# mandanasmi/lane-slam

Hardware: AMD Instinct MI355X
Metric: frames/sec (640x480) detect->descript->project->sanity->associate (higher is better)
Workload: dtype u8/f64 (FP4 e2m1 MFMA with exact f32 accumulation for association)

## Files before the change

### include/lanefront.h

```cpp
#ifndef LANEFRONT_H
#define LANEFRONT_H

#include <stddef.h>
#include <stdint.h>

#define LF_API __attribute__((visibility("default")))

#ifdef __cplusplus
extern "C" {
#endif

#define LF_ABI_VERSION 5

typedef enum lf_status {
    LF_OK = 0,
    LF_ERR_BAD_ARG = -1,
    LF_ERR_CAPACITY = -2,
    LF_ERR_HIP = -3,
    LF_ERR_NOT_INITIALISED = -4,
    LF_ERR_UNSUPPORTED = -5,
    LF_ERR_DECODE = -6
} lf_status;

#define LF_WHITE 0
// ... 399 lines not shown
LF_API int lf_jpeg_decode_batch_gpu_async(lf_handle* h, const uint8_t* const* jpeg, const size_t* jpeg_size, int n_frames,
                                   int rows, int cols, uint8_t* frames_device, int n_threads);
LF_API int lf_jpeg_status(lf_handle* h, int* frame_status, int n_frames, int* n_failed);
LF_API int lf_jpeg_decode_for_detect_async(lf_handle* h, const uint8_t* const* jpeg, const size_t* jpeg_size, int n_frames, int n_threads);
LF_API int lf_jpeg_info(const uint8_t* jpeg, size_t jpeg_size, int* rows, int* cols, int* components, int* hmax, int* vmax);
LF_API int lf_frames_buffer(lf_handle* h, uint8_t** device_ptr, size_t* bytes);

#define LF_MSG_DETECTOR 0
#define LF_MSG_GROUND 1
#define LF_MSG_FILTERED 2
LF_API int lf_serialize_segments(lf_handle* h, const lf_segments* segs, int segs_on_device, int n_frames, int stage,
                          uint8_t* out, size_t out_capacity, int out_on_device, int64_t* frame_byte_offset);
LF_API int lf_deserialize_segments(lf_handle* h, const uint8_t* bodies, int bodies_on_device, const int64_t* frame_byte_offset,
                            int n_frames, lf_segments* out, int out_on_device, int* n_segments);

LF_API int lf_draw_lines(lf_handle* h, int n_frames, const lf_segments* seg, int seg_on_device, uint8_t* out_bgr, int out_on_device);
LF_API int lf_draw_lines_image(lf_handle* h, const uint8_t* bgr, int n_frames, int rows, int cols, const lf_segments* seg, int seg_on_device,
                               uint8_t* out_bgr, int images_on_device);

#define LF_JPEG_ENCODE_STAGES 8
LF_API size_t lf_jpeg_encode_bound(int rows, int cols);
LF_API int lf_jpeg_encode_batch(lf_handle* h, const uint8_t* bgr, int bgr_on_device, int n_frames, int rows, int cols, int quality, uint8_t* out,
                                size_t out_stride, uint32_t* out_size, int out_on_device);
LF_API int lf_jpeg_encode_timing(lf_handle* h, double* ms_per_stage, int n);
LF_API const char* lf_jpeg_encode_stage_name(int stage);

#define LF_RECTIFY_STAGES 1
LF_API int lf_set_camera(lf_handle* h, const double* K, const double* D, const double* R, const double* P, int cam_w, int cam_h);
LF_API int lf_set_rectified_input(lf_handle* h, int flag);
LF_API int lf_get_rectified_input(lf_handle* h, int* flag);
LF_API int lf_rectify_map(lf_handle* h, float* mapx, float* mapy);
LF_API int lf_rectify_batch(lf_handle* h, const uint8_t* src, int src_on_device, int n_frames, int rows, int cols, int channels, uint8_t* dst,
                            int dst_on_device);
LF_API int lf_rectify_timing(lf_handle* h, double* ms_per_stage, int n);
LF_API const char* lf_rectify_stage_name(int stage);

typedef enum lf_buffer_id {
    LF_BUF_BGR = 0,
    LF_BUF_MASKS = 1,
    LF_BUF_EDGES = 2,
    LF_BUF_LSD_ANGLE = 3,
    LF_BUF_LSD_MODGRAD = 4,
    LF_BUF_LSD_ORDER = 5,
    LF_BUF_LSD_NORDER = 6,
    LF_BUF_LBD_DX = 7,
    LF_BUF_LBD_DY = 8,
    LF_BUF_LSD_COUNTS = 9,
    LF_BUF_LSD_SCRATCH = 10,
    LF_BUF_LSD_NLOW = 11
} lf_buffer_id;
LF_API int lf_debug_fetch(lf_handle* h, int buffer_id, void* dst, size_t bytes);
LF_API int lf_debug_detmath(lf_handle* h, int which, const double* a, const double* b_or_null, double* y, int n);
LF_API int lf_debug_probe(lf_handle* h, int width, int write, size_t bytes, int reps);
LF_API int lf_debug_lsd_binary(lf_handle* h, const uint8_t* img, int rows, int cols, float* lines4, int cap, int* n_out);
LF_API int lf_debug_std_sort(lf_handle* h, const int32_t* keys, int n, int32_t* order);
LF_API int lf_lsd_size(const lf_handle* h, int* rows, int* cols);
LF_API int lf_suggested_depth(const lf_handle* h);

LF_API int lf_lsd_list_capacity(const lf_handle* h, int* entries, int* grown);
LF_API int lf_lsd_scratch_stride(const lf_handle* h);

#define LF_N_STAGES 16
LF_API int lf_set_profiling(lf_handle* h, int enabled);
LF_API int lf_get_timing(lf_handle* h, double* ms_per_stage, int32_t* launches_per_stage, int n);
LF_API int lf_reset_timing(lf_handle* h);
LF_API const char* lf_stage_name(int stage);

#ifdef __cplusplus
}
#endif
#endif
```

### lane_slam_amd/_lib.py

```python
import ctypes
import os

from .config import LfConfig

_HERE = os.path.dirname(os.path.abspath(__file__))
SO_PATH = os.environ.get("LANEFRONT_LIBRARY") or os.path.join(_HERE, "liblanefront.so")

LF_N_STAGES = 16
LF_MAP_N_STAGES = 4
LF_MSG_DETECTOR, LF_MSG_GROUND, LF_MSG_FILTERED = 0, 1, 2
(LF_BUF_BGR, LF_BUF_MASKS, LF_BUF_EDGES, LF_BUF_LSD_ANGLE, LF_BUF_LSD_MODGRAD, LF_BUF_LSD_ORDER,
 LF_BUF_LSD_NORDER, LF_BUF_LBD_DX, LF_BUF_LBD_DY, LF_BUF_LSD_COUNTS, LF_BUF_LSD_SCRATCH, LF_BUF_LSD_NLOW) = range(12)

EXPORTS = (
    "lf_abi_version", "lf_create", "lf_destroy", "lf_last_error", "lf_synchronize", "lf_get_stream",
    "lf_set_image", "lf_detect_lines", "lf_process_batch", "lf_process_batch_async", "lf_wait", "lf_associate", "lf_associate_float", "lf_kmeans",
    "lf_jpeg_decode_batch", "lf_jpeg_info", "lf_frames_buffer", "lf_serialize_segments", "lf_deserialize_segments",
    "lf_debug_fetch", "lf_debug_detmath", "lf_debug_probe", "lf_debug_lsd_binary", "lf_lsd_size", "lf_set_profiling", "lf_get_timing", "lf_reset_timing", "lf_stage_name",
    "lf_map_create", "lf_map_destroy", "lf_map_last_error", "lf_map_get_stream", "lf_map_synchronize", "lf_map_seed", "lf_map_size",
    "lf_map_associate", "lf_map_pack_block", "lf_map_update", "lf_map_step", "lf_map_step_host", "lf_map_fetch",
    "lf_map_set_profiling", "lf_map_get_timing", "lf_map_stage_name",
    "lf_descriptor_default_params", "lf_set_descriptor_params", "lf_get_descriptor_params",
    "lf_edlines_default_params", "lf_keylines_batch", "lf_describe_keylines", "lf_keylines_debug_fetch", "lf_set_image_edlines", "lf_knn_match", "lf_radius_match", "lf_jpeg_decode_batch_gpu", "lf_jpeg_decode_batch_gpu_async", "lf_jpeg_status", "lf_jpeg_decode_for_detect_async",
    "lf_set_tie_rule", "lf_map_set_tie_rule", "lf_debug_std_sort", "lf_suggested_depth", "lf_lsd_list_capacity", "lf_lsd_scratch_stride", "lf_set_detector", "lf_detector_failures", "lf_keylines_batch_async", "lf_keylines_frame_status", "lf_lsd_keylines_batch", "lf_select_queries",
    "lf_lsd_default_options", "lf_lsd_keylines_batch_ex", "lf_keylines_batch_masked",
    "lf_matcher_add", "lf_matcher_clear", "lf_matcher_size", "lf_matcher_match", "lf_matcher_knn_match", "lf_matcher_radius_match",
    "lf_lane_filter_default_config", "lf_lane_filter_create", "lf_lane_filter_destroy", "lf_lane_filter_last_error", "lf_lane_filter_grid",
    "lf_lane_filter_set_tables", "lf_lane_filter_reset", "lf_lane_filter_step", "lf_lane_filter_get_poses", "lf_lane_filter_get_belief",
    "lf_lane_filter_synchronize", "lf_lane_filter_set_profiling", "lf_lane_filter_get_timing", "lf_lane_filter_stage_name",
    "lf_hough_default_params", "lf_set_hough_params", "lf_get_hough_params",
    "lf_dense_default_params", "lf_set_dense_params", "lf_get_dense_params",
    "lf_ai_transform_batch", "lf_set_ai_transform", "lf_get_ai_transform",
    "lf_draw_lines", "lf_draw_lines_image",
    "lf_jpeg_encode_bound", "lf_jpeg_encode_batch", "lf_jpeg_encode_timing", "lf_jpeg_encode_stage_name",
    "lf_set_camera", "lf_set_rectified_input", "lf_get_rectified_input", "lf_rectify_map", "lf_rectify_batch", "lf_rectify_timing",
    "lf_rectify_stage_name",
    "lf_map_default_view", "lf_map_bounds", "lf_map_render", "lf_map_render_counts", "lf_map_render_timing", "lf_map_render_stage_name",
    "lf_sizeof_camera_view", "lf_map_camera_view", "lf_map_render_camera", "lf_map_render_camera_timing",
    "lf_sizeof_align_config", "lf_sizeof_align_result", "lf_map_align_default_config", "lf_map_align", "lf_map_step_aligned",
    "lf_map_step_aligned_host", "lf_map_align_timing",
    "lf_sizeof_smooth_config", "lf_map_smooth_default_config", "lf_map_smooth", "lf_map_step_smoothed", "lf_map_step_smoothed_host",
    "lf_map_smooth_timing",
    "lf_sizeof_localize_config", "lf_sizeof_localize_result", "lf_map_localize_default_config", "lf_map_localize", "lf_map_localize_timing",
    "lf_sizeof_prune_config", "lf_sizeof_prune_result", "lf_map_prune_default_config", "lf_map_prune", "lf_map_prune_timing",
)
LF_ALIGN_OK, LF_ALIGN_FEW, LF_ALIGN_DEGENERATE, LF_ALIGN_REJECTED = 0, 1, 2, 3
ALIGN_STATUS = ("ok", "few", "degenerate", "rejected")
LF_MAP_RENDER_STAGES = 4
LF_JPEG_ENCODE_STAGES = 8
LF_RECTIFY_STAGES = 1
LF_LANE_FILTER_PREDICT, LF_LANE_FILTER_UPDATE = 1, 2
LF_LANE_FILTER_MAX_CELLS = 4096
LF_LANE_FILTER_N_STAGES = 2
LANE_FILTER_PARAMS = ("mean_d_0", "mean_phi_0", "sigma_d_0", "sigma_phi_0", "delta_d", "delta_phi", "d_max", "d_min", "phi_max",
                      "phi_min", "cov_v", "linewidth_white", "linewidth_yellow", "lanewidth", "min_max", "sigma_d_mask", "sigma_phi_mask")
DETECTORS = {"lsd": 0, "edlines": 1, "hough": 2, "dense": 3}
HOUGH_KEYS = ("hough_threshold", "hough_min_line_length", "hough_max_line_gap")
DENSE_KEYS = ("sobel_threshold",)
TIE_RULES = {"lowest": 0, "mihasher": 1}
LF_MAX_OCTAVES = 5


class LfSegments(ctypes.Structure):
    _fields_ = [
        ("capacity", ctypes.c_int32),
        ("frame_offset", ctypes.c_void_p),
        ("lines", ctypes.c_void_p), ("normals", ctypes.c_void_p), ("color", ctypes.c_void_p),
        ("pixels_normalized", ctypes.c_void_p), ("ground", ctypes.c_void_p), ("keep", ctypes.c_void_p),
        ("desc", ctypes.c_void_p), ("code", ctypes.c_void_p),
    ]

# ... 146 lines not shown
    lib.lf_process_batch_async.restype = ci
    lib.lf_wait.argtypes = [vp, ctypes.POINTER(ci)]
    lib.lf_wait.restype = ci
    lib.lf_associate.argtypes = [vp, vp, ci, vp, ci, vp, vp, ci]
    lib.lf_associate_float.argtypes = [vp, vp, ci, vp, ci, vp, vp, ci]
    lib.lf_kmeans.argtypes = [vp, vp, ci, ci, ci, vp, ci, ctypes.c_double, vp, vp, vp, vp]
    lib.lf_ai_transform_batch.argtypes = [vp, vp, ci, ci, ci, ci, vp]
    lib.lf_set_ai_transform.argtypes = [vp, vp, vp]
    lib.lf_get_ai_transform.argtypes = [vp, vp, vp]
    lib.lf_draw_lines.argtypes = [vp, ci, ctypes.POINTER(LfSegments), ci, vp, ci]
    lib.lf_draw_lines_image.argtypes = [vp, vp, ci, ci, ci, ctypes.POINTER(LfSegments), ci, vp, ci]
    lib.lf_jpeg_encode_bound.argtypes = [ci, ci]
    lib.lf_jpeg_encode_bound.restype = ctypes.c_size_t
    lib.lf_jpeg_encode_batch.argtypes = [vp, vp, ci, ci, ci, ci, ci, vp, ctypes.c_size_t, vp, ci]
    lib.lf_jpeg_encode_batch.restype = ci
    lib.lf_jpeg_encode_timing.argtypes = [vp, vp, ci]
    lib.lf_jpeg_encode_timing.restype = ci
    lib.lf_jpeg_encode_stage_name.argtypes = [ci]
    lib.lf_jpeg_encode_stage_name.restype = ctypes.c_char_p
    lib.lf_set_camera.argtypes = [vp, vp, vp, vp, vp, ci, ci]
    lib.lf_set_rectified_input.argtypes = [vp, ci]
    lib.lf_get_rectified_input.argtypes = [vp, ctypes.POINTER(ci)]
    lib.lf_rectify_map.argtypes = [vp, vp, vp]
    lib.lf_rectify_batch.argtypes = [vp, vp, ci, ci, ci, ci, ci, vp, ci]
    lib.lf_rectify_timing.argtypes = [vp, vp, ci]
    for f in ("lf_set_camera", "lf_set_rectified_input", "lf_get_rectified_input", "lf_rectify_map", "lf_rectify_batch", "lf_rectify_timing"):
        getattr(lib, f).restype = ci
    lib.lf_rectify_stage_name.argtypes = [ci]
    lib.lf_rectify_stage_name.restype = ctypes.c_char_p
    lib.lf_jpeg_decode_batch.argtypes = [vp, ctypes.POINTER(vp), ctypes.POINTER(ctypes.c_size_t), ci, ci, ci, vp, ci, ci,
                                         ctypes.POINTER(ci)]
    lib.lf_jpeg_decode_batch.restype = ci
    lib.lf_jpeg_decode_batch_gpu.argtypes = lib.lf_jpeg_decode_batch.argtypes
    lib.lf_jpeg_decode_batch_gpu.restype = ci
    lib.lf_jpeg_decode_batch_gpu_async.argtypes = [vp, ctypes.POINTER(vp), ctypes.POINTER(ctypes.c_size_t), ci, ci, ci, vp, ci]
    lib.lf_jpeg_decode_batch_gpu_async.restype = ci
    lib.lf_jpeg_status.argtypes = [vp, ctypes.POINTER(ci), ci, ctypes.POINTER(ci)]
    lib.lf_jpeg_decode_for_detect_async.argtypes = [vp, ctypes.POINTER(vp), ctypes.POINTER(ctypes.c_size_t), ci, ci]
    lib.lf_jpeg_decode_for_detect_async.restype = ci
    lib.lf_jpeg_status.restype = ci
    lib.lf_jpeg_info.argtypes = [vp, ctypes.c_size_t] + [ctypes.POINTER(ci)] * 5
    lib.lf_jpeg_info.restype = ci
    lib.lf_frames_buffer.argtypes = [vp, ctypes.POINTER(vp), ctypes.POINTER(ctypes.c_size_t)]
    lib.lf_frames_buffer.restype = ci
    lib.lf_serialize_segments.argtypes = [vp, ctypes.POINTER(LfSegments), ci, ci, ci, vp, ctypes.c_size_t, ci,
                                          ctypes.POINTER(ctypes.c_int64)]
    lib.lf_serialize_segments.restype = ci
    lib.lf_deserialize_segments.argtypes = [vp, vp, ci, ctypes.POINTER(ctypes.c_int64), ci, ctypes.POINTER(LfSegments), ci,
                                            ctypes.POINTER(ci)]
    lib.lf_deserialize_segments.restype = ci
    lib.lf_debug_fetch.argtypes = [vp, ci, vp, ctypes.c_size_t]
    lib.lf_debug_detmath.argtypes = [vp, ci, vp, vp, vp, ci]
    lib.lf_debug_detmath.restype = ci
    lib.lf_debug_probe.argtypes = [vp, ci, ci, ctypes.c_size_t, ci]
    lib.lf_debug_probe.restype = ci
    lib.lf_debug_lsd_binary.argtypes = [vp, vp, ci, ci, vp, ci, ctypes.POINTER(ci)]
    lib.lf_debug_lsd_binary.restype = ci
    lib.lf_lsd_size.argtypes = [vp, ctypes.POINTER(ci), ctypes.POINTER(ci)]
    lib.lf_set_profiling.argtypes = [vp, ci]
    lib.lf_get_timing.argtypes = [vp, vp, vp, ci]
    lib.lf_reset_timing.argtypes = [vp]
    lib.lf_stage_name.argtypes = [ci]
    lib.lf_stage_name.restype = ctypes.c_char_p
    i64p = ctypes.POINTER(ctypes.c_int64)
    lib.lf_map_create.argtypes = [ci, ctypes.POINTER(LfMapConfig), ctypes.POINTER(vp)]
    lib.lf_map_destroy.argtypes = [vp]
    lib.lf_map_destroy.restype = None
    lib.lf_map_last_error.argtypes = [vp]
    lib.lf_map_last_error.restype = ctypes.c_char_p
    lib.lf_map_get_stream.argtypes = [vp, ctypes.POINTER(vp)]
    lib.lf_map_synchronize.argtypes = [vp]
    lib.lf_map_seed.argtypes = [vp, vp, vp, vp, ci, ci]
    lib.lf_map_size.argtypes = [vp, ctypes.POINTER(ci), ctypes.POINTER(ci), i64p, i64p]
    lib.lf_map_associate.argtypes = [vp, vp, vp, vp, ci, vp, vp, ci]
    lib.lf_map_pack_block.argtypes = [vp, vp, ctypes.POINTER(LfSegments), ci, ci, vp, vp, vp, ci, vp, ci]
    lib.lf_map_update.argtypes = [vp, vp, ci, ci]
    lib.lf_map_step.argtypes = [vp, vp, ctypes.POINTER(LfSegments), ci, ci, vp, ci, vp, vp]
    lib.lf_map_step_host.argtypes = [vp, ctypes.POINTER(LfSegments), ci, ci, vp, ci, vp, vp]
    lib.lf_map_step_host.restype = ci
    lib.lf_map_fetch.argtypes = [vp, ci, ci, vp, vp, vp, vp, vp]
    lib.lf_map_set_profiling.argtypes = [vp, ci]
    lib.lf_map_set_profiling.restype = ci
    lib.lf_map_get_timing.argtypes = [vp, vp, vp, ci]
    lib.lf_map_get_timing.restype = ci
    lib.lf_map_stage_name.argtypes = [ci]
    lib.lf_map_stage_name.restype = ctypes.c_char_p
    lib.lf_map_default_view.argtypes = [ctypes.POINTER(LfMapView)]
    lib.lf_map_default_view.restype = None
    lib.lf_map_bounds.argtypes = [vp, ctypes.POINTER(LfMapView), vp, ctypes.POINTER(ci)]
    lib.lf_map_render.argtypes = [vp, ctypes.POINTER(LfMapView), vp, ci, vp, ci, ctypes.POINTER(ci), ctypes.POINTER(ci)]
    lib.lf_map_render_counts.argtypes = [vp, ctypes.POINTER(ci), ctypes.POINTER(ci)]
    lib.lf_map_render_timing.argtypes = [vp, vp, ci]
    for f in ("lf_map_bounds", "lf_map_render", "lf_map_render_counts", "lf_map_render_timing"):
        getattr(lib, f).restype = ci
    lib.lf_map_render_stage_name.argtypes = [ci]
    lib.lf_map_render_stage_name.restype = ctypes.c_char_p
    lib.lf_sizeof_camera_view.argtypes = []
    lib.lf_map_camera_view.argtypes = [vp, ci, ci, ci, ci, ci, ctypes.POINTER(LfCameraView)]
    lib.lf_map_render_camera.argtypes = [vp, ctypes.POINTER(LfCameraView), vp, ci, vp, vp, ci, vp]
    lib.lf_map_render_camera_timing.argtypes = [vp, vp, ci]
    for f in ("lf_sizeof_camera_view", "lf_map_camera_view", "lf_map_render_camera", "lf_map_render_camera_timing"):
        getattr(lib, f).restype = ci
    lib.lf_sizeof_align_config.argtypes = []
    lib.lf_sizeof_align_result.argtypes = []
    lib.lf_map_align_default_config.argtypes = [ctypes.POINTER(LfAlignConfig)]
    lib.lf_map_align_default_config.restype = None
# ... 137 lines not shown
```

### lane_slam_amd/csrc/k_canny.hip

```cpp
#include "common.h"

namespace lf {

#ifndef LF_CANNY_ROWS
#define LF_CANNY_ROWS 62
#endif
constexpr int CB_R = LF_CANNY_ROWS;
static_assert(CB_R + 2 <= 64, "the columns beside a strip are worked out with one lane per magnitude row");

typedef short cn_s2 __attribute__((ext_vector_type(2)));

struct CannyH {
    cn_s2 d_br, s_br;
    int d_g, s_g;
};
struct CannyG {
    cn_s2 dx_br, dy_br;
    int dx_g, dy_g;
    uint32_t m_br;
    int m_g;
};

__device__ __forceinline__ cn_s2 canny_a_plus_2b(cn_s2 a, cn_s2 b)
{
    cn_s2 d;
    const uint32_t two = 0x00020002u;
    asm("v_pk_mad_i16 %0, %1, %2, %3" : "=v"(d) : "v"(b), "v"(two), "v"(a));
    return d;
}

__device__ __forceinline__ CannyH canny_hterms(uint32_t aL, uint32_t aM, uint32_t aR)
{
    const cn_s2 l = __builtin_bit_cast(cn_s2, aL & 0x00ff00ffu), m = __builtin_bit_cast(cn_s2, aM & 0x00ff00ffu), r = __builtin_bit_cast(cn_s2, aR & 0x00ff00ffu);
    const int lg = (int)((aL >> 8) & 0xffu), mg = (int)((aM >> 8) & 0xffu), rg = (int)((aR >> 8) & 0xffu);
    CannyH h;
    h.d_br = r - l;
    h.s_br = canny_a_plus_2b(l, m) + r;
    h.d_g = rg - lg;
    h.s_g = lg + 2 * mg + rg;
    return h;
}

__device__ __forceinline__ int canny_mag_at(const uint32_t* __restrict__ img, int W, int Hc, int x, int y)
{
    if (x < 0 || x >= W || y < 0 || y >= Hc) return 0;
    const int xl = max(x - 1, 0), xr = min(x + 1, W - 1), yu = max(y - 1, 0), yd = min(y + 1, Hc - 1);
    const uint32_t a00 = img[(size_t)yu * W + xl], a01 = img[(size_t)yu * W + x], a02 = img[(size_t)yu * W + xr];
    const uint32_t a10 = img[(size_t)y * W + xl], a12 = img[(size_t)y * W + xr];
    const uint32_t a20 = img[(size_t)yd * W + xl], a21 = img[(size_t)yd * W + x], a22 = img[(size_t)yd * W + xr];
    int best = 0;
#pragma unroll
    for (int ch = 0; ch < 3; ++ch) {
        const int sh = 8 * ch;
        const int v00 = (a00 >> sh) & 255, v01 = (a01 >> sh) & 255, v02 = (a02 >> sh) & 255, v10 = (a10 >> sh) & 255, v12 = (a12 >> sh) & 255;
        const int v20 = (a20 >> sh) & 255, v21 = (a21 >> sh) & 255, v22 = (a22 >> sh) & 255;
        const int dx = (v02 - v00) + 2 * (v12 - v10) + (v22 - v20);
        const int dy = (v20 - v00) + 2 * (v21 - v01) + (v22 - v02);
        best = max(best, abs(dx) + abs(dy));
    }
    return best;
}

__device__ __forceinline__ int canny_from_left(int v, int edge) { return __builtin_amdgcn_update_dpp(edge, v, 0x138, 0xf, 0xf, false); }
__device__ __forceinline__ int canny_from_right(int v, int edge) { return __builtin_amdgcn_update_dpp(edge, v, 0x130, 0xf, 0xf, false); }

struct CannyBand {
    const uint32_t* img;
    __amdgpu_buffer_rsrc_t rsrc;
    __amdgpu_buffer_rsrc_t rs_weak, rs_strong;
    int W, Hc, Ww, low, high;
    int x0, y0, y_end;
    uint32_t xl, xm, xr;
    int lane;
    bool in_image;
    bool st_ok;
    uint32_t st_off;
    int* halo;
};

__device__ __forceinline__ void canny_fetch(const CannyBand& c, int prow, uint32_t (&px)[3])
{
    const int yy = min(max(prow, 0), c.Hc - 1);
    const int row = yy * c.W * 4;
    px[0] = __builtin_amdgcn_raw_buffer_load_b32(c.rsrc, (int)c.xl, row, 0);
    px[1] = __builtin_amdgcn_raw_buffer_load_b32(c.rsrc, (int)c.xm, row, 0);
    px[2] = __builtin_amdgcn_raw_buffer_load_b32(c.rsrc, (int)c.xr, row, 0);
}

__device__ __forceinline__ void canny_halo_chunk(const CannyBand& c, int t)
{
    const int side = c.lane >> 5, j = t - 4 + (c.lane & 31);
    if ((c.lane & 31) < 18 && j >= 0 && j < 64)
        c.halo[side * 64 + j] = canny_mag_at(c.img, c.W, c.Hc, side ? c.x0 + 64 : c.x0 - 1, c.y0 - 1 + j);
    __builtin_amdgcn_fence(__ATOMIC_RELEASE, "wavefront");
    __builtin_amdgcn_wave_barrier();
}

template <int A, int B, int C>
__device__ __forceinline__ void canny_step(const CannyBand& c, int t, uint32_t (&px)[3][3], CannyH (&H)[3], int (&M)[3], CannyG (&G)[3])
{
    const int p = c.y0 - 2 + t;
    if ((t & 15) == 0) canny_halo_chunk(c, t);
    H[C] = canny_hterms(px[C][0], px[C][1], px[C][2]);
    canny_fetch(c, p + 3, px[C]);
    if (t < 2) return;
    {
        const int y = p - 1;
        const cn_s2 zero = { 0, 0 };
        CannyG g;
        g.dx_br = canny_a_plus_2b(H[A].d_br, H[B].d_br) + H[C].d_br;
        g.dy_br = H[C].s_br - H[A].s_br;
        g.dx_g = H[A].d_g + 2 * H[B].d_g + H[C].d_g;
        g.dy_g = H[C].s_g - H[A].s_g;
        const cn_s2 m_br = __builtin_elementwise_max(g.dx_br, zero - g.dx_br) + __builtin_elementwise_max(g.dy_br, zero - g.dy_br);
        g.m_g = abs(g.dx_g) + abs(g.dy_g);
        g.m_br = __builtin_bit_cast(uint32_t, m_br);
        const int best = max(max((int)(g.m_br & 0xffffu), (int)(g.m_br >> 16)), g.m_g);
        M[C] = (c.in_image && y >= 0 && y < c.Hc) ? best : 0;
        G[C] = g;
    }
    const int yn = p - 2;
    if (yn < c.y0 || yn >= c.y_end) return;
    const int m = M[B];
    const unsigned long long over = __ballot(m > c.low);
    unsigned long long keep = 0ull, hi = 0ull;
    if (over != 0ull) {
        const int* hl = c.halo + (yn - c.y0 + 1);
        const int up = M[A], dn = M[C];
        const int mL = canny_from_left(m, hl[0]), mR = canny_from_right(m, hl[64]);
        const int upL = canny_from_left(up, hl[-1]), upR = canny_from_right(up, hl[63]);
        const int dnL = canny_from_left(dn, hl[1]), dnR = canny_from_right(dn, hl[65]);
        const CannyG g = G[B];
        const int m_b = (int)(g.m_br & 0xffffu), m_r = (int)(g.m_br >> 16);
        const bool take_g = g.m_g > m_b;
        const bool take_r = m_r > max(m_b, g.m_g);
        const int xs = take_r ? (int)g.dx_br.y : (take_g ? g.dx_g : (int)g.dx_br.x);
        const int ys = take_r ? (int)g.dy_br.y : (take_g ? g.dy_g : (int)g.dy_br.x);
        const int TG22 = (int)(0.4142135623730950488016887242097 * (1 << 15) + 0.5);
        const int ax = abs(xs), ay = abs(ys) << 15;
        int tg22x;
        asm("v_mul_u32_u24 %0, %1, %2" : "=v"(tg22x) : "v"(ax), "v"(TG22));
        const int tg67x = tg22x + (ax << 16);
        const bool neg = (xs ^ ys) < 0;
        const unsigned long long keep_h = __ballot(m > mL) & __ballot(m >= mR);
        const unsigned long long keep_v = __ballot(m > up) & __ballot(m >= dn);
        const unsigned long long keep_d = __ballot(m > (neg ? upR : upL)) & __ballot(m > (neg ? dnL : dnR));
        const unsigned long long is_h = __ballot(ay < tg22x), is_v = __ballot(ay > tg67x) & ~is_h;
        keep = over & ((is_h & keep_h) | (is_v & keep_v) | (~(is_h | is_v) & keep_d));
        hi = keep & __ballot(m > c.high);
    }
    if (c.st_ok) {
        const int o = (yn * c.Ww + (c.x0 >> 5)) * 4;
        const bool second = c.lane != 0;
        __builtin_amdgcn_raw_buffer_store_b32(second ? (uint32_t)(keep >> 32) : (uint32_t)keep, c.rs_weak, (int)c.st_off, o, 0);
        __builtin_amdgcn_raw_buffer_store_b32(second ? (uint32_t)(hi >> 32) : (uint32_t)hi, c.rs_strong, (int)c.st_off, o, 0);
    }
}

#ifndef LF_CANNY_WAVES
#define LF_CANNY_WAVES 7
#endif
__global__ __launch_bounds__(256) __attribute__((amdgpu_waves_per_eu(LF_CANNY_WAVES, LF_CANNY_WAVES))) void k_canny_nms(CannyParams p, int n_units, int n_strips, int n_bands,
                                                   const uint32_t* __restrict__ bgr, uint32_t* __restrict__ strong,
                                                   uint32_t* __restrict__ weak)
{
    __shared__ int halo[4][128];
    int b = (int)blockIdx.x;
    {
        const int per_frame = (n_strips * n_bands + 3) / 4;
        const int full = (n_units / (n_strips * n_bands)) / 8 * 8 * per_frame;
        if (b < full) {
            const int grp = b / (8 * per_frame), r = b - grp * 8 * per_frame;
            b = (grp * 8 + (r & 7)) * per_frame + (r >> 3);
        }
    }
    const int wave = __builtin_amdgcn_readfirstlane((int)(threadIdx.x >> 6));
    const int per_frame_u = n_strips * n_bands, wg_per_frame = (per_frame_u + 3) / 4;
    const int f = b / wg_per_frame, uf = (b - f * wg_per_frame) * 4 + wave;
    if (uf >= per_frame_u || f * per_frame_u >= n_units) return;
    const int u = uf;
    CannyBand c;
    c.lane = (int)(threadIdx.x & 63u);
    const int strip = u % n_strips, band = u / n_strips;
    c.W = p.W; c.Hc = p.Hc; c.Ww = p.Ww; c.low = p.low; c.high = p.high;
    c.img = bgr + (size_t)f * p.Hc * p.W;
    c.rsrc = __builtin_amdgcn_make_buffer_rsrc(const_cast<uint32_t*>(c.img), 0, p.Hc * p.W * 4, 0x00020000);
    c.rs_weak = __builtin_amdgcn_make_buffer_rsrc(weak + (size_t)f * p.Hc * p.Ww, 0, p.Hc * p.Ww * 4, 0x00020000);
    c.rs_strong = __builtin_amdgcn_make_buffer_rsrc(strong + (size_t)f * p.Hc * p.Ww, 0, p.Hc * p.Ww * 4, 0x00020000);
    c.x0 = strip * 64; c.y0 = band * CB_R; c.y_end = min(c.y0 + CB_R, p.Hc);
    const int x = c.x0 + c.lane;
    c.in_image = x < p.W;
    c.st_ok = c.lane < 2 && (c.x0 >> 5) + c.lane < p.Ww;
    c.st_off = 4u * (uint32_t)c.lane;
    const int xm = min(x, p.W - 1);
    c.xm = 4u * (uint32_t)xm; c.xl = 4u * (uint32_t)max(xm - 1, 0); c.xr = 4u * (uint32_t)min(xm + 1, p.W - 1);
    c.halo = halo[threadIdx.x >> 6];
    uint32_t px[3][3];
    CannyH H[3];
    int M[3] = { 0, 0, 0 };
    CannyG G[3];
    canny_fetch(c, c.y0 - 2, px[0]);
    canny_fetch(c, c.y0 - 1, px[1]);
    canny_fetch(c, c.y0, px[2]);
    const int steps = (c.y_end - c.y0) + 4;
    for (int t = 0; t < steps; t += 3) {
        canny_step<1, 2, 0>(c, t, px, H, M, G);
        canny_step<2, 0, 1>(c, t + 1, px, H, M, G);
        canny_step<0, 1, 2>(c, t + 2, px, H, M, G);
    }
}

void launch_canny(const CannyParams& p, const uint32_t* bgr, int n_frames, uint32_t* strong, uint32_t* weak,
                  hipStream_t s)
{
    const int n_strips = (p.W + 63) / 64, n_bands = (p.Hc + CB_R - 1) / CB_R;
    const int n_units = n_strips * n_bands * n_frames;
    const int wg_per_frame = (n_strips * n_bands + 3) / 4;
    hipLaunchKernelGGL(k_canny_nms, dim3(wg_per_frame * n_frames), dim3(256), 0, s, p, n_units, n_strips, n_bands, bgr, strong, weak);
}

__device__ __forceinline__ uint32_t fill_up(uint32_t w, uint32_t s) { return (((w + s) ^ w) & w) | s; }

__global__ __launch_bounds__(1024) void k_hysteresis(CannyParams p, uint32_t* __restrict__ strong,
                                                      const uint32_t* __restrict__ weak)
{
    extern __shared__ uint32_t lds[];
    const int nw = p.Hc * p.Ww;
    uint32_t* S = lds;
    uint32_t* Wk = lds + nw;
    const int f = blockIdx.x;
    uint32_t* gs = strong + (size_t)f * nw;
    const uint32_t* gw = weak + (size_t)f * nw;
    for (int i = threadIdx.x; i < nw; i += blockDim.x) { S[i] = gs[i]; Wk[i] = gw[i]; }
    __syncthreads();
    const int Ww = p.Ww;
    for (int iter = 0; iter < 65536; ++iter) {
        int changed = 0;
        uint32_t upd[8];
#pragma unroll
        for (int cnt = 0; cnt < 8; ++cnt) {
            const int i = threadIdx.x + cnt * 1024;
            upd[cnt] = 0;
            if (i >= nw) continue;
            int y = i / Ww, x = i - y * Ww;
            uint32_t w = Wk[i];
            uint32_t cur = S[i];
            uint32_t acc = 0;
            if (w) {
#pragma unroll
                for (int dy = -1; dy <= 1; ++dy) {
                    int yy = y + dy;
                    if (yy < 0 || yy >= p.Hc) continue;
                    const uint32_t* row = S + yy * Ww;
                    uint32_t c = row[x];
                    uint32_t l = x > 0 ? row[x - 1] : 0u;
                    uint32_t r = x + 1 < Ww ? row[x + 1] : 0u;
                    acc |= c | (c << 1) | (c >> 1) | (l >> 31) | (r << 31);
                }
                uint32_t s = acc & w;
                s = fill_up(w, s);
                s = __brev(fill_up(__brev(w), __brev(s)));
// ... 214 lines not shown
```

### lane_slam_amd/csrc/k_debug.hip

```cpp
#include "common.h"

namespace lf {

__global__ void k_detmath(int which, const double* __restrict__ a, const double* __restrict__ b,
                          double* __restrict__ y, int n)
{
    int i = blockIdx.x * blockDim.x + threadIdx.x;
    if (i >= n) return;
    double x = a[i], z = b ? b[i] : 0.0, r = 0.0;
    switch (which) {
    case 0: r = dm::dexp(x); break;
    case 1: r = dm::dlog(x); break;
    case 2: r = dm::dsin(x); break;
    case 3: r = dm::dcos(x); break;
    case 4: r = dm::datan(x); break;
    case 5: r = dm::dasin(x); break;
    case 6: r = dm::dlog10(x); break;
    case 7: r = dm::dsinh_small(x); break;
    case 8: r = dm::datan2(x, z); break;
    case 9: r = dm::dpow(x, z); break;
    case 10: r = dm::dsqrt(x); break;
    case 11: r = x / z; break;
    case 12: r = (double)dm::fast_atan2_deg((float)x, (float)z); break;
    case 13: r = (double)dm::fsqrt((float)x); break;
    case 14: r = (double)dm::fdiv((float)x, (float)z); break;
    default: r = 0.0;
    }
    y[i] = r;
}

template <int W>
__global__ void k_probe_read(const uint32_t* __restrict__ src, size_t n_words, uint32_t* __restrict__ sink)
{
    constexpr int D = W / 4;
    uint32_t acc = 0;
    const size_t stride = (size_t)gridDim.x * blockDim.x * D;
    for (size_t i = ((size_t)blockIdx.x * blockDim.x + threadIdx.x) * D; i + D <= n_words; i += stride) {
        if (D == 1) acc ^= src[i];
        else if (D == 2) { const uint2 v = *reinterpret_cast<const uint2*>(src + i); acc ^= v.x ^ v.y; }
        else if (D == 3) { acc ^= src[i] ^ src[i + 1] ^ src[i + 2]; }
        else { const uint4 v = *reinterpret_cast<const uint4*>(src + i); acc ^= v.x ^ v.y ^ v.z ^ v.w; }
    }
    if (acc == 0x9e3779b9u) sink[0] = acc;
}

template <int W>
__global__ void k_probe_write(uint32_t* __restrict__ dst, size_t n_words)
{
    constexpr int D = W / 4;
    const size_t stride = (size_t)gridDim.x * blockDim.x * D;
    for (size_t i = ((size_t)blockIdx.x * blockDim.x + threadIdx.x) * D; i + D <= n_words; i += stride) {
        if (D == 1) dst[i] = (uint32_t)i;
        else *reinterpret_cast<uint4*>(dst + i) = make_uint4((uint32_t)i, 1u, 2u, 3u);
// ... 19 lines not shown
    if (acc == 0x9e3779b9u) sink[0] = acc;
}

}

extern "C" int lf_debug_probe(lf_handle* h, int width, int write, size_t bytes, int reps)
{
    if (!h || bytes < 4096 || reps < 1) return LF_ERR_BAD_ARG;
    uint32_t *buf = nullptr, *sink = nullptr;
    if (hipMalloc((void**)&buf, bytes) != hipSuccess || hipMalloc((void**)&sink, 256) != hipSuccess) {
        if (buf) (void)hipFree(buf);
        lf_set_error(h, LF_ERR_HIP, "lf_debug_probe: hipMalloc failed");
        return LF_ERR_HIP;
    }
    (void)hipMemset(buf, 1, bytes);
    const size_t nw = bytes / 4;
    const dim3 grid(256 * 16), block(256);
    for (int r = 0; r < reps; ++r) {
        if (write) {
            if (width == 4) hipLaunchKernelGGL(lf::k_probe_write<4>, grid, block, 0, 0, buf, nw);
            else hipLaunchKernelGGL(lf::k_probe_write<16>, grid, block, 0, 0, buf, nw);
        } else if (width == 43) {
            const int nf = (int)(bytes / (640 * 320 * 4));
            hipLaunchKernelGGL(lf::k_probe_stencil, dim3((nf * 60 + 3) / 4), block, 0, 0, buf, nf, sink);
        } else if (width == 4) hipLaunchKernelGGL(lf::k_probe_read<4>, grid, block, 0, 0, buf, nw, sink);
        else if (width == 8) hipLaunchKernelGGL(lf::k_probe_read<8>, grid, block, 0, 0, buf, nw, sink);
        else if (width == 12) hipLaunchKernelGGL(lf::k_probe_read<12>, grid, block, 0, 0, buf, nw, sink);
        else hipLaunchKernelGGL(lf::k_probe_read<16>, grid, block, 0, 0, buf, nw, sink);
    }
    const hipError_t e = hipDeviceSynchronize();
    (void)hipFree(buf); (void)hipFree(sink);
    if (e != hipSuccess) { lf_set_error(h, LF_ERR_HIP, "lf_debug_probe: %s", hipGetErrorString(e)); return LF_ERR_HIP; }
    return LF_OK;
}

extern "C" int lf_debug_detmath(lf_handle* h, int which, const double* a, const double* b, double* y, int n)
{
    if (!h || !a || !y || n <= 0) return LF_ERR_BAD_ARG;
    double *da = nullptr, *db = nullptr, *dy = nullptr;
    size_t bytes = (size_t)n * sizeof(double);
    if (hipMalloc((void**)&da, bytes) != hipSuccess || hipMalloc((void**)&db, bytes) != hipSuccess ||
        hipMalloc((void**)&dy, bytes) != hipSuccess) {
        lf_set_error(h, LF_ERR_HIP, "lf_debug_detmath: hipMalloc failed");
        return LF_ERR_HIP;
    }
    (void)hipMemcpy(da, a, bytes, hipMemcpyHostToDevice);
    if (b) (void)hipMemcpy(db, b, bytes, hipMemcpyHostToDevice);
    hipLaunchKernelGGL(lf::k_detmath, dim3((n + 255) / 256), dim3(256), 0, 0, which, da, b ? db : nullptr, dy, n);
    hipError_t e = hipMemcpy(y, dy, bytes, hipMemcpyDeviceToHost);
    (void)hipFree(da); (void)hipFree(db); (void)hipFree(dy);
    if (e != hipSuccess) { lf_set_error(h, LF_ERR_HIP, "lf_debug_detmath: %s", hipGetErrorString(e)); return LF_ERR_HIP; }
    return LF_OK;
}
```

Before: 114,300.

## Defer Canny non-max suppression to a compacted LDS candidate queue with ring buffer

The Canny kernel used to run non-maximum suppression for every row with wave-wide ballots over DPP neighbour shuffles. It now writes gradient magnitudes into a 16-row LDS ring and pushes only above-low-threshold pixels into a compacted 64-entry LDS queue. The queue is drained in batches, looking up exactly two neighbours per candidate, and edge bits are set with LDS atomics. Weak/strong masks are written once per band at the end instead of once per row, which adds LDS use per workgroup and extra wave syncs. A debug entry point for running Canny alone is also added.

New measurement: 113,700. No clear change (-0.5%).

```diff
diff --git a/include/lanefront.h b/include/lanefront.h
--- a/include/lanefront.h
+++ b/include/lanefront.h
@@ -475,6 +475,7 @@
 LF_API int lf_debug_fetch(lf_handle* h, int buffer_id, void* dst, size_t bytes);
 LF_API int lf_debug_detmath(lf_handle* h, int which, const double* a, const double* b_or_null, double* y, int n);
 LF_API int lf_debug_probe(lf_handle* h, int width, int write, size_t bytes, int reps);
+LF_API int lf_debug_canny(lf_handle* h, const uint8_t* bgr, int n, int rows, int cols, double lo, double hi, uint8_t* edges);
 LF_API int lf_debug_lsd_binary(lf_handle* h, const uint8_t* img, int rows, int cols, float* lines4, int cap, int* n_out);
 LF_API int lf_debug_std_sort(lf_handle* h, const int32_t* keys, int n, int32_t* order);
 LF_API int lf_lsd_size(const lf_handle* h, int* rows, int* cols);
diff --git a/lane_slam_amd/_lib.py b/lane_slam_amd/_lib.py
--- a/lane_slam_amd/_lib.py
+++ b/lane_slam_amd/_lib.py
@@ -16,7 +16,7 @@
     "lf_abi_version", "lf_create", "lf_destroy", "lf_last_error", "lf_synchronize", "lf_get_stream",
     "lf_set_image", "lf_detect_lines", "lf_process_batch", "lf_process_batch_async", "lf_wait", "lf_associate", "lf_associate_float", "lf_kmeans",
     "lf_jpeg_decode_batch", "lf_jpeg_info", "lf_frames_buffer", "lf_serialize_segments", "lf_deserialize_segments",
-    "lf_debug_fetch", "lf_debug_detmath", "lf_debug_probe", "lf_debug_lsd_binary", "lf_lsd_size", "lf_set_profiling", "lf_get_timing", "lf_reset_timing", "lf_stage_name",
+    "lf_debug_fetch", "lf_debug_detmath", "lf_debug_probe", "lf_debug_canny", "lf_debug_lsd_binary", "lf_lsd_size", "lf_set_profiling", "lf_get_timing", "lf_reset_timing", "lf_stage_name",
     "lf_map_create", "lf_map_destroy", "lf_map_last_error", "lf_map_get_stream", "lf_map_synchronize", "lf_map_seed", "lf_map_size",
     "lf_map_associate", "lf_map_pack_block", "lf_map_update", "lf_map_step", "lf_map_step_host", "lf_map_fetch",
     "lf_map_set_profiling", "lf_map_get_timing", "lf_map_stage_name",
@@ -269,6 +269,8 @@
     lib.lf_debug_fetch.argtypes = [vp, ci, vp, ctypes.c_size_t]
     lib.lf_debug_detmath.argtypes = [vp, ci, vp, vp, vp, ci]
     lib.lf_debug_detmath.restype = ci
+    lib.lf_debug_canny.argtypes = [vp, vp, ci, ci, ci, ctypes.c_double, ctypes.c_double, vp]
+    lib.lf_debug_canny.restype = ci
     lib.lf_debug_probe.argtypes = [vp, ci, ci, ctypes.c_size_t, ci]
     lib.lf_debug_probe.restype = ci
     lib.lf_debug_lsd_binary.argtypes = [vp, vp, ci, ci, vp, ci, ctypes.POINTER(ci)]
diff --git a/lane_slam_amd/csrc/k_canny.hip b/lane_slam_amd/csrc/k_canny.hip
--- a/lane_slam_amd/csrc/k_canny.hip
+++ b/lane_slam_amd/csrc/k_canny.hip
@@ -14,12 +14,23 @@
     cn_s2 d_br, s_br;
     int d_g, s_g;
 };
-struct CannyG {
-    cn_s2 dx_br, dy_br;
-    int dx_g, dy_g;
+
+constexpr int CN_RING = 16;
+constexpr int CN_STRIDE = 68;
+constexpr int CN_QUEUE = 64;
+constexpr int CN_AGE = CN_RING - 2;
+struct CannyRec {
+    uint32_t dx_br, dy_br;
+    uint32_t g;
     uint32_t m_br;
-    int m_g;
 };
+struct __attribute__((aligned(16))) CannyLds {
+    CannyRec q[CN_QUEUE];
+    uint32_t out[64][4];
+    uint16_t ring[CN_RING][CN_STRIDE];
+    uint16_t halo[2][64];
+};
+static_assert(sizeof(CannyLds) == 4480, "17.5 KB per workgroup: seven workgroups and one of region growing (25 KB) share a CU's 160 KB");
 
 __device__ __forceinline__ cn_s2 canny_a_plus_2b(cn_s2 a, cn_s2 b)
 {
@@ -61,100 +72,140 @@
     return best;
 }
 
-__device__ __forceinline__ int canny_from_left(int v, int edge) { return __builtin_amdgcn_update_dpp(edge, v, 0x138, 0xf, 0xf, false); }
-__device__ __forceinline__ int canny_from_right(int v, int edge) { return __builtin_amdgcn_update_dpp(edge, v, 0x130, 0xf, 0xf, false); }
-
 struct CannyBand {
     const uint32_t* img;
     __amdgpu_buffer_rsrc_t rsrc;
-    __amdgpu_buffer_rsrc_t rs_weak, rs_strong;
-    int W, Hc, Ww, low, high;
-    int x0, y0, y_end;
+    int W, Hc, low, high;
+    int x0, y0, rows;
+    int row_off, row_pitch, row_last;
     uint32_t xl, xm, xr;
     int lane;
+    uint32_t lane_tag;
     bool in_image;
-    bool st_ok;
-    uint32_t st_off;
-    int* halo;
+    CannyLds* lds;
+    int pending, deadline;
 };
 
-__device__ __forceinline__ void canny_fetch(const CannyBand& c, int prow, uint32_t (&px)[3])
-{
-    const int yy = min(max(prow, 0), c.Hc - 1);
-    const int row = yy * c.W * 4;
+__device__ __forceinline__ void canny_fetch(const CannyBand& c, int row, uint32_t (&px)[3])
+{
     px[0] = __builtin_amdgcn_raw_buffer_load_b32(c.rsrc, (int)c.xl, row, 0);
     px[1] = __builtin_amdgcn_raw_buffer_load_b32(c.rsrc, (int)c.xm, row, 0);
     px[2] = __builtin_amdgcn_raw_buffer_load_b32(c.rsrc, (int)c.xr, row, 0);
 }
 
+__device__ __forceinline__ void canny_wave_sync()
+{
+    __builtin_amdgcn_fence(__ATOMIC_RELEASE, "wavefront");
+    __builtin_amdgcn_wave_barrier();
+    __builtin_amdgcn_fence(__ATOMIC_ACQUIRE, "wavefront");
+}
+
 __device__ __forceinline__ void canny_halo_chunk(const CannyBand& c, int t)
 {
     const int side = c.lane >> 5, j = t - 4 + (c.lane & 31);
     if ((c.lane & 31) < 18 && j >= 0 && j < 64)
-        c.halo[side * 64 + j] = canny_mag_at(c.img, c.W, c.Hc, side ? c.x0 + 64 : c.x0 - 1, c.y0 - 1 + j);
-    __builtin_amdgcn_fence(__ATOMIC_RELEASE, "wavefront");
-    __builtin_amdgcn_wave_barrier();
-}
-
-template <int A, int B, int C>
-__device__ __forceinline__ void canny_step(const CannyBand& c, int t, uint32_t (&px)[3][3], CannyH (&H)[3], int (&M)[3], CannyG (&G)[3])
-{
-    const int p = c.y0 - 2 + t;
-    if ((t & 15) == 0) canny_halo_chunk(c, t);
-    H[C] = canny_hterms(px[C][0], px[C][1], px[C][2]);
-    canny_fetch(c, p + 3, px[C]);
-    if (t < 2) return;
-    {
-        const int y = p - 1;
-        const cn_s2 zero = { 0, 0 };
-        CannyG g;
-        g.dx_br = canny_a_plus_2b(H[A].d_br, H[B].d_br) + H[C].d_br;
-        g.dy_br = H[C].s_br - H[A].s_br;
-        g.dx_g = H[A].d_g + 2 * H[B].d_g + H[C].d_g;
-        g.dy_g = H[C].s_g - H[A].s_g;
-        const cn_s2 m_br = __builtin_elementwise_max(g.dx_br, zero - g.dx_br) + __builtin_elementwise_max(g.dy_br, zero - g.dy_br);
-        g.m_g = abs(g.dx_g) + abs(g.dy_g);
-        g.m_br = __builtin_bit_cast(uint32_t, m_br);
-        const int best = max(max((int)(g.m_br & 0xffffu), (int)(g.m_br >> 16)), g.m_g);
-        M[C] = (c.in_image && y >= 0 && y < c.Hc) ? best : 0;
-        G[C] = g;
-    }
-    const int yn = p - 2;
-    if (yn < c.y0 || yn >= c.y_end) return;
-    const int m = M[B];
-    const unsigned long long over = __ballot(m > c.low);
-    unsigned long long keep = 0ull, hi = 0ull;
-    if (over != 0ull) {
-        const int* hl = c.halo + (yn - c.y0 + 1);
-        const int up = M[A], dn = M[C];
-        const int mL = canny_from_left(m, hl[0]), mR = canny_from_right(m, hl[64]);
-        const int upL = canny_from_left(up, hl[-1]), upR = canny_from_right(up, hl[63]);
-        const int dnL = canny_from_left(dn, hl[1]), dnR = canny_from_right(dn, hl[65]);
-        const CannyG g = G[B];
-        const int m_b = (int)(g.m_br & 0xffffu), m_r = (int)(g.m_br >> 16);
-        const bool take_g = g.m_g > m_b;
-        const bool take_r = m_r > max(m_b, g.m_g);
-        const int xs = take_r ? (int)g.dx_br.y : (take_g ? g.dx_g : (int)g.dx_br.x);
-        const int ys = take_r ? (int)g.dy_br.y : (take_g ? g.dy_g : (int)g.dy_br.x);
+        c.lds->halo[side][j] = (uint16_t)canny_mag_at(c.img, c.W, c.Hc, side ? c.x0 + 64 : c.x0 - 1, c.y0 - 1 + j);
+    canny_wave_sync();
+}
+
+__device__ __forceinline__ void canny_decide(CannyBand& c, int jc)
+{
+    CannyLds* L = c.lds;
+    if (c.lane < 2 * CN_RING) {
+        const int s = c.lane & (CN_RING - 1), side = c.lane >> 4;
+        const int js = jc - ((jc - s) & (CN_RING - 1));
+        if (js >= 0) L->ring[s][side ? 65 : 0] = L->halo[side][js];
+    }
+    canny_wave_sync();
+    if (c.lane < c.pending) {
+        const CannyRec r = L->q[c.lane];
+        const cn_s2 dx_br = __builtin_bit_cast(cn_s2, r.dx_br), dy_br = __builtin_bit_cast(cn_s2, r.dy_br);
+        const int dx_g = (int)(r.g << 21) >> 21, dy_g = (int)r.g >> 21;
+        const int col = (int)(r.g >> 11) & 63, s = (int)(r.g >> 17) & (CN_RING - 1);
+        const int m_b = (int)(r.m_br & 0xffffu), m_r = (int)(r.m_br >> 16), m_g = abs(dx_g) + abs(dy_g);
+        const int m = max(max(m_b, m_r), m_g);
+        const bool take_g = m_g > m_b;
+        const bool take_r = m_r > max(m_b, m_g);
+        const int xs = take_r ? (int)dx_br.y : (take_g ? dx_g : (int)dx_br.x);
+        const int ys = take_r ? (int)dy_br.y : (take_g ? dy_g : (int)dy_br.x);
         const int TG22 = (int)(0.4142135623730950488016887242097 * (1 << 15) + 0.5);
         const int ax = abs(xs), ay = abs(ys) << 15;
         int tg22x;
         asm("v_mul_u32_u24 %0, %1, %2" : "=v"(tg22x) : "v"(ax), "v"(TG22));
         const int tg67x = tg22x + (ax << 16);
         const bool neg = (xs ^ ys) < 0;
-        const unsigned long long keep_h = __ballot(m > mL) & __ballot(m >= mR);
-        const unsigned long long keep_v = __ballot(m > up) & __ballot(m >= dn);
-        const unsigned long long keep_d = __ballot(m > (neg ? upR : upL)) & __ballot(m > (neg ? dnL : dnR));
-        const unsigned long long is_h = __ballot(ay < tg22x), is_v = __ballot(ay > tg67x) & ~is_h;
-        keep = over & ((is_h & keep_h) | (is_v & keep_v) | (~(is_h | is_v) & keep_d));
-        hi = keep & __ballot(m > c.high);
-    }
-    if (c.st_ok) {
-        const int o = (yn * c.Ww + (c.x0 >> 5)) * 4;
-        const bool second = c.lane != 0;
-        __builtin_amdgcn_raw_buffer_store_b32(second ? (uint32_t)(keep >> 32) : (uint32_t)keep, c.rs_weak, (int)c.st_off, o, 0);
-        __builtin_amdgcn_raw_buffer_store_b32(second ? (uint32_t)(hi >> 32) : (uint32_t)hi, c.rs_strong, (int)c.st_off, o, 0);
-    }
+        const bool is_h = ay < tg22x, is_v = !is_h && ay > tg67x;
+        const int ox = is_v ? 0 : ((!is_h && neg) ? 1 : -1), oy = is_h ? 0 : -1;
+        const uint16_t* ring = &L->ring[0][0];
+        const int n1 = ring[((s + oy) & (CN_RING - 1)) * CN_STRIDE + col + 1 + ox];
+        const int n2 = ring[((s - oy) & (CN_RING - 1)) * CN_STRIDE + col + 1 - ox];
+        if (m > n1 && m + ((is_h || is_v) ? 1 : 0) > n2) {
+            const int row = jc - ((jc - s) & (CN_RING - 1)) - 1;
+            const uint32_t bit = 1u << (col & 31);
+            atomicOr(&L->out[row][col >> 5], bit);
+            if (m > c.high) atomicOr(&L->out[row][2 + (col >> 5)], bit);
+        }
+    }
+    canny_wave_sync();
+    c.pending = 0;
+    c.deadline = 1 << 20;
+}
+
+struct CannyG {
+    cn_s2 dx_br, dy_br;
+    int dx_g, dy_g;
+    uint32_t m_br;
+    int best;
+};
+
+__device__ __forceinline__ CannyG canny_gradient(const CannyH& a, const CannyH& b, const CannyH& c)
+{
+    const cn_s2 zero = { 0, 0 };
+    CannyG g;
+    g.dx_br = canny_a_plus_2b(a.d_br, b.d_br) + c.d_br;
+    g.dy_br = c.s_br - a.s_br;
+    g.dx_g = a.d_g + 2 * b.d_g + c.d_g;
+    g.dy_g = c.s_g - a.s_g;
+    g.m_br = __builtin_bit_cast(uint32_t, __builtin_elementwise_max(g.dx_br, zero - g.dx_br) + __builtin_elementwise_max(g.dy_br, zero - g.dy_br));
+    g.best = max(max((int)(g.m_br & 0xffffu), (int)(g.m_br >> 16)), abs(g.dx_g) + abs(g.dy_g));
+    return g;
+}
+
+template <int A, int B, int C>
+__device__ __forceinline__ void canny_step(CannyBand& c, int t, uint32_t (&px)[3][3], CannyH (&H)[3])
+{
+    if ((t & 15) == 0) canny_halo_chunk(c, t);
+    H[C] = canny_hterms(px[C][0], px[C][1], px[C][2]);
+    canny_fetch(c, c.row_off, px[C]);
+    c.row_off = min(c.row_off + c.row_pitch, c.row_last);
+    const int j = t - 2;
+    uint16_t* ring = &c.lds->ring[j & (CN_RING - 1)][1 + c.lane];
+    if ((unsigned)(j - 1) >= (unsigned)c.rows) {
+        if (j == 0 || j == c.rows + 1) {
+            const int y = c.y0 - 1 + j;
+            *ring = (uint16_t)((c.in_image && y >= 0 && y < c.Hc) ? canny_gradient(H[A], H[B], H[C]).best : 0);
+        }
+        return;
+    }
+    const CannyG g = canny_gradient(H[A], H[B], H[C]);
+    const int m = c.in_image ? g.best : 0;
+    *ring = (uint16_t)m;
+    const bool cand = m > c.low;
+    const unsigned long long over = __ballot(cand);
+    const int n = __builtin_popcountll(over);
+    if (c.pending + n > CN_QUEUE || j >= c.deadline) canny_decide(c, j);
+    if (n == 0) return;
+    if (c.pending == 0) c.deadline = j + CN_AGE;
+    if (cand) {
+        const uint32_t pos = __builtin_amdgcn_mbcnt_hi((uint32_t)(over >> 32), __builtin_amdgcn_mbcnt_lo((uint32_t)over, (uint32_t)c.pending));
+        CannyRec r;
+        r.dx_br = __builtin_bit_cast(uint32_t, g.dx_br);
+        r.dy_br = __builtin_bit_cast(uint32_t, g.dy_br);
+        r.g = ((uint32_t)g.dx_g & 0x7ffu) | c.lane_tag | ((uint32_t)(j & (CN_RING - 1)) << 17) | ((uint32_t)g.dy_g << 21);
+        r.m_br = g.m_br;
+        c.lds->q[pos] = r;
+    }
+    c.pending += n;
 }
 
 #ifndef LF_CANNY_WAVES
@@ -164,7 +215,7 @@
                                                    const uint32_t* __restrict__ bgr, uint32_t* __restrict__ strong,
                                                    uint32_t* __restrict__ weak)
 {
-    __shared__ int halo[4][128];
+    __shared__ CannyLds lds[4];
     int b = (int)blockIdx.x;
     {
         const int per_frame = (n_strips * n_bands + 3) / 4;
@@ -181,32 +232,45 @@
     const int u = uf;
     CannyBand c;
     c.lane = (int)(threadIdx.x & 63u);
+    c.lane_tag = (uint32_t)c.lane << 11;
     const int strip = u % n_strips, band = u / n_strips;
-    c.W = p.W; c.Hc = p.Hc; c.Ww = p.Ww; c.low = p.low; c.high = p.high;
+    c.W = p.W; c.Hc = p.Hc; c.low = p.low; c.high = p.high;
     c.img = bgr + (size_t)f * p.Hc * p.W;
     c.rsrc = __builtin_amdgcn_make_buffer_rsrc(const_cast<uint32_t*>(c.img), 0, p.Hc * p.W * 4, 0x00020000);
-    c.rs_weak = __builtin_amdgcn_make_buffer_rsrc(weak + (size_t)f * p.Hc * p.Ww, 0, p.Hc * p.Ww * 4, 0x00020000);
-    c.rs_strong = __builtin_amdgcn_make_buffer_rsrc(strong + (size_t)f * p.Hc * p.Ww, 0, p.Hc * p.Ww * 4, 0x00020000);
-    c.x0 = strip * 64; c.y0 = band * CB_R; c.y_end = min(c.y0 + CB_R, p.Hc);
+    c.x0 = strip * 64; c.y0 = band * CB_R; c.rows = min(CB_R, p.Hc - c.y0);
+    c.row_pitch = p.W * 4; c.row_last = (p.Hc - 1) * c.row_pitch;
     const int x = c.x0 + c.lane;
     c.in_image = x < p.W;
-    c.st_ok = c.lane < 2 && (c.x0 >> 5) + c.lane < p.Ww;
-    c.st_off = 4u * (uint32_t)c.lane;
     const int xm = min(x, p.W - 1);
     c.xm = 4u * (uint32_t)xm; c.xl = 4u * (uint32_t)max(xm - 1, 0); c.xr = 4u * (uint32_t)min(xm + 1, p.W - 1);
-    c.halo = halo[threadIdx.x >> 6];
+    c.lds = &lds[wave];
+    c.pending = 0; c.deadline = 1 << 20;
+    *reinterpret_cast<uint4*>(c.lds->out[c.lane]) = make_uint4(0u, 0u, 0u, 0u);
     uint32_t px[3][3];
     CannyH H[3];
-    int M[3] = { 0, 0, 0 };
-    CannyG G[3];
-    canny_fetch(c, c.y0 - 2, px[0]);
-    canny_fetch(c, c.y0 - 1, px[1]);
-    canny_fetch(c, c.y0, px[2]);
-    const int steps = (c.y_end - c.y0) + 4;
+    canny_fetch(c, max(c.y0 - 2, 0) * c.row_pitch, px[0]);
+    canny_fetch(c, max(c.y0 - 1, 0) * c.row_pitch, px[1]);
+    canny_fetch(c, c.y0 * c.row_pitch, px[2]);
+    c.row_off = min((c.y0 + 1) * c.row_pitch, c.row_last);
+    const int steps = c.rows + 4;
     for (int t = 0; t < steps; t += 3) {
-        canny_step<1, 2, 0>(c, t, px, H, M, G);
-        canny_step<2, 0, 1>(c, t + 1, px, H, M, G);
-        canny_step<0, 1, 2>(c, t + 2, px, H, M, G);
+        canny_step<1, 2, 0>(c, t, px, H);
+        canny_step<2, 0, 1>(c, t + 1, px, H);
+        canny_step<0, 1, 2>(c, t + 2, px, H);
+    }
+    if (c.pending != 0) canny_decide(c, c.rows + 1);
+    else canny_wave_sync();
+    if (c.lane < c.rows) {
+        const uint4 o = *reinterpret_cast<const uint4*>(c.lds->out[c.lane]);
+        const __amdgpu_buffer_rsrc_t rs_weak = __builtin_amdgcn_make_buffer_rsrc(weak + (size_t)f * p.Hc * p.Ww, 0, p.Hc * p.Ww * 4, 0x00020000);
+        const __amdgpu_buffer_rsrc_t rs_strong = __builtin_amdgcn_make_buffer_rsrc(strong + (size_t)f * p.Hc * p.Ww, 0, p.Hc * p.Ww * 4, 0x00020000);
+        const int at = ((c.y0 + c.lane) * p.Ww + (c.x0 >> 5)) * 4;
+        __builtin_amdgcn_raw_buffer_store_b32(o.x, rs_weak, at, 0, 0);
+        __builtin_amdgcn_raw_buffer_store_b32(o.z, rs_strong, at, 0, 0);
+        if ((c.x0 >> 5) + 1 < p.Ww) {
+            __builtin_amdgcn_raw_buffer_store_b32(o.y, rs_weak, at + 4, 0, 0);
+            __builtin_amdgcn_raw_buffer_store_b32(o.w, rs_strong, at + 4, 0, 0);
+        }
     }
 }
 
diff --git a/lane_slam_amd/csrc/k_debug.hip b/lane_slam_amd/csrc/k_debug.hip
--- a/lane_slam_amd/csrc/k_debug.hip
+++ b/lane_slam_amd/csrc/k_debug.hip
@@ -1,4 +1,5 @@
 #include "common.h"
+#include <vector>
 
 namespace lf {
 
@@ -124,3 +125,38 @@
     if (e != hipSuccess) { lf_set_error(h, LF_ERR_HIP, "lf_debug_detmath: %s", hipGetErrorString(e)); return LF_ERR_HIP; }
     return LF_OK;
 }
+
+extern "C" int lf_debug_canny(lf_handle* h, const uint8_t* bgr, int n, int rows, int cols, double lo, double hi, uint8_t* edges)
+{
+    if (!h || !bgr || !edges || n <= 0 || rows <= 0 || cols <= 0) return LF_ERR_BAD_ARG;
+    lf::CannyParams p;
+    p.Hc = rows; p.W = cols; p.Ww = (cols + 31) / 32;
+    if (lo > hi) { const double t = lo; lo = hi; hi = t; }
+    p.low = lf::dm::ifloor(lo); p.high = lf::dm::ifloor(hi);
+    const size_t npix = (size_t)n * rows * cols, plane = (size_t)n * rows * p.Ww * sizeof(uint32_t);
+    std::vector<uint32_t> bgrx(npix);
+    for (size_t i = 0; i < npix; ++i) bgrx[i] = (uint32_t)bgr[3 * i] | (uint32_t)bgr[3 * i + 1] << 8 | (uint32_t)bgr[3 * i + 2] << 16;
+    uint32_t *d_bgrx = nullptr, *d_strong = nullptr, *d_weak = nullptr;
+    uint8_t* d_edges = nullptr;
+    hipError_t e = hipMalloc((void**)&d_bgrx, npix * 4);
+    if (e == hipSuccess) e = hipMalloc((void**)&d_strong, plane);
+    if (e == hipSuccess) e = hipMalloc((void**)&d_weak, plane);
+    if (e == hipSuccess) e = hipMalloc((void**)&d_edges, npix);
+    if (e == hipSuccess) e = hipMemcpy(d_bgrx, bgrx.data(), npix * 4, hipMemcpyHostToDevice);
+    int rc = LF_OK;
+    if (e == hipSuccess) {
+        lf::launch_canny(p, d_bgrx, n, d_strong, d_weak, 0);
+        if (lf::launch_hysteresis(p, n, d_strong, d_weak, 0) != 0) rc = LF_ERR_UNSUPPORTED;
+        else {
+            lf::launch_edges_u8(p, n, d_strong, d_edges, 0);
+            e = hipMemcpy(edges, d_edges, npix, hipMemcpyDeviceToHost);
+        }
+    }
+    if (d_bgrx) (void)hipFree(d_bgrx);
+    if (d_strong) (void)hipFree(d_strong);
+    if (d_weak) (void)hipFree(d_weak);
+    if (d_edges) (void)hipFree(d_edges);
+    if (e != hipSuccess) { lf_set_error(h, LF_ERR_HIP, "lf_debug_canny: %s", hipGetErrorString(e)); return LF_ERR_HIP; }
+    if (rc != LF_OK) lf_set_error(h, rc, "lf_debug_canny: a %dx%d image does not fit the hysteresis strips", rows, cols);
+    return rc;
+}
```
